# Tarseus/eam-rl4co

Measured on AMD Instinct MI355X. Metric: env-steps/sec (batch x num_loc / s), AttentionModel construction rollout, higher is better.
Workload: dtype f32; 1 GPU; TSP num_loc=100 batch=1024/GPU AM greedy rollout (encoder + cache + decode loop + reward); global_batch=1024, launch=hipGraph replay

## Files before the change

eam_rl4co_amd/csrc/encoder_fused.hip:

```cpp
#include "encoder_fused.hpp"

namespace eamrl {

constexpr int SA = 140;
constexpr int GA = 34;
constexpr int SQ = 66;

struct ALayout {
    float* HB;
    static constexpr int S = SA;
    __device__ float* col(int c) const { return HB + (c & 3) * GA + (c >> 2); }
    __device__ void store4(int row, int q4, float4 v) const
    {
        float* p = HB + row * SA + q4;
        p[0] = v.x; p[GA] = v.y; p[2 * GA] = v.z; p[3 * GA] = v.w;
    }
    __device__ float4 load4(int row, int q4) const
    {
        const float* p = HB + row * SA + q4;
        return make_float4(p[0], p[GA], p[2 * GA], p[3 * GA]);
    }
    __device__ void mirror(int, int, float) const {}
};

#ifdef EAMRL_STAMPS
__device__ unsigned long long g_enc_stamps[24];
#define ESTAMP(i) do { const unsigned long long now_ = __builtin_readcyclecounter(); st_acc[i] += now_ - st_t; st_t = now_; } while (0)
#else
#define ESTAMP(i) do { } while (0)
#endif

__device__ __forceinline__ f32x4 mfma4(float a, float b, f32x4 c) { return __builtin_amdgcn_mfma_f32_16x16x4f32(a, b, c, 0, 0, 0); }

typedef float f32x2v __attribute__((ext_vector_type(2)));
__device__ __forceinline__ float2 lds_read_b64(const float* p)
{
    typedef const volatile __attribute__((address_space(3))) f32x2v* lds_ptr;
    const f32x2v v = *(lds_ptr)(p);
    return make_float2(v.x, v.y);
}

template <int CT>
__device__ __forceinline__ void load_b0(float4 (&b0)[CT], const float* const (&wp)[CT])
{
#pragma unroll
    for (int ct = 0; ct < CT; ++ct) b0[ct] = *reinterpret_cast<const float4*>(wp[ct]);
}

template <int RTW, int CT, int S, bool SWAP, int NRT>
__device__ __forceinline__ void gemm_pass_n(f32x4 (&acc)[RTW][CT], const float* arow, const float* const (&wp)[CT],
                                            int NU, const float4 (&b0)[CT])
{
    constexpr int nrt = NRT;
    float4 bn[CT];
    float2 an0[RTW], an1[RTW];
#pragma unroll
    for (int ct = 0; ct < CT; ++ct) bn[ct] = b0[ct];
#pragma unroll
    for (int rt = 0; rt < RTW; ++rt)
        if (rt < nrt) {
            an0[rt] = lds_read_b64(arow + rt * 16 * S);
            an1[rt] = lds_read_b64(arow + rt * 16 * S + 2);
        }
    for (int u = 0; u < NU; ++u) {
        float4 b[CT];
        float2 a0[RTW], a1[RTW];
#pragma unroll
        for (int ct = 0; ct < CT; ++ct) b[ct] = bn[ct];
#pragma unroll
        for (int rt = 0; rt < RTW; ++rt) { a0[rt] = an0[rt]; a1[rt] = an1[rt]; }
        if (u + 1 < NU) {
#pragma unroll
            for (int ct = 0; ct < CT; ++ct) bn[ct] = *reinterpret_cast<const float4*>(wp[ct] + (u + 1) * 256);
#pragma unroll
            for (int rt = 0; rt < RTW; ++rt)
                if (rt < nrt) {
                    an0[rt] = lds_read_b64(arow + rt * 16 * S + 4 * (u + 1));
                    an1[rt] = lds_read_b64(arow + rt * 16 * S + 4 * (u + 1) + 2);
                }
        }
#pragma unroll
        for (int rt = 0; rt < RTW; ++rt)
            if (rt < nrt) {
#pragma unroll
                for (int ct = 0; ct < CT; ++ct)
                    acc[rt][ct] = SWAP ? mfma4(b[ct].x, a0[rt].x, acc[rt][ct]) : mfma4(a0[rt].x, b[ct].x, acc[rt][ct]);
#pragma unroll
                for (int ct = 0; ct < CT; ++ct)
                    acc[rt][ct] = SWAP ? mfma4(b[ct].y, a0[rt].y, acc[rt][ct]) : mfma4(a0[rt].y, b[ct].y, acc[rt][ct]);
#pragma unroll
                for (int ct = 0; ct < CT; ++ct)
                    acc[rt][ct] = SWAP ? mfma4(b[ct].z, a1[rt].x, acc[rt][ct]) : mfma4(a1[rt].x, b[ct].z, acc[rt][ct]);
#pragma unroll
                for (int ct = 0; ct < CT; ++ct)
                    acc[rt][ct] = SWAP ? mfma4(b[ct].w, a1[rt].y, acc[rt][ct]) : mfma4(a1[rt].y, b[ct].w, acc[rt][ct]);
            }
    }
}

template <int RTW, int CT, int S, bool SWAP = false, int NLOW = RTW>
__device__ __forceinline__ void gemm_pass(f32x4 (&acc)[RTW][CT], const float* arow, int nrt, const float* const (&wp)[CT],
                                          int NU, const float4 (&b0)[CT])
{
    if (NLOW == RTW || nrt == RTW) gemm_pass_n<RTW, CT, S, SWAP, RTW>(acc, arow, wp, NU, b0);
    else gemm_pass_n<RTW, CT, S, SWAP, NLOW>(acc, arow, wp, NU, b0);
}

template <int RTW>
__device__ __forceinline__ void residual_norm_store(const f32x4 (&acc)[RTW][2], float* HB, int row0, int nrt, int cw, int j, int G,
                                                    int norm, const float* cst )
{
#pragma unroll
    for (int ct = 0; ct < 2; ++ct) {
        const int c = 32 * cw + 16 * ct + j;
        const float sc = cst[c], sh = cst[FE + c];
        float* col = HB + (c & 3) * GA + (c >> 2);
#pragma unroll
        for (int rt = 0; rt < RTW; ++rt)
            if (rt < nrt) {
#pragma unroll
                for (int r = 0; r < 4; ++r) {
                    float* p = col + (row0 + 16 * rt + 4 * G + r) * SA;
                    float v = *p + acc[rt][ct][r];
                    if (norm == EAMRL_NORM_BATCH_EVAL) v = fma_(v, sc, sh);
                    *p = v;
                }
            }
    }
}

template <int RTT>
__global__ __launch_bounds__(512, 2) void k_encoder_fused(FusedArgs a)
{
    constexpr int RTA = (RTT + 1) / 2;
    constexpr int RTW = RTA;
    constexpr int ROWS = 16 * RTT;
    constexpr int SV = ROWS + 4;
    extern __shared__ __attribute__((aligned(16))) float lds[];
    float* HB = lds;
    float* QA = HB + ROWS * SA;
    float* KB = QA + ROWS * SQ;
    float* VT = KB + ROWS * SQ;
    float* HID = QA;
    float* CST = VT + 64 * SV;
    static_assert(ROWS * SA <= 2 * ROWS * SQ + 64 * SV, "HID must fit QA | KB | VT");
    const ALayout L{HB};

    const int tid = threadIdx.x, lane = tid & 63;
    const int wv = __builtin_amdgcn_readfirstlane(tid >> 6);
    const int cw = wv & 3, rw = wv >> 2;
    const int j = lane & 15, G = lane >> 4;
    const int M = a.M;
    const int row0 = rw ? 16 * RTA : 0;
    const int nrt = rw ? RTT - RTA : RTA;
    const int64_t inst = blockIdx.x;
#ifdef EAMRL_STAMPS
    unsigned long long st_acc[20] = {0, 0, 0, 0, 0, 0, 0, 0, 0, 0, 0, 0, 0, 0, 0, 0, 0, 0, 0, 0}, st_t = __builtin_readcyclecounter();
#endif

    if (a.h_in) load_h<ROWS>(a.h_in, M, L);
    else init_embedding<ROWS>(a.init, M, L);
    __syncthreads();
    ESTAMP(0);

    for (int layer = 0; layer < a.nlayers; ++layer) {
        const eamrl_encoder_layer& Ly = a.L[layer];
        for (int i = tid; i < NCST; i += blockDim.x) {
            float v;
            if (i < C_BO) v = Ly.bqkv[i];
            else if (i < C_B1) v = Ly.bo[i - C_BO];
            else if (i < C_B2) v = Ly.b1[i - C_B1];
            else if (i < C_N1) v = Ly.b2[i - C_B2];
            else {
                const bool second = i >= C_N2;
                const int k = (i - (second ? C_N2 : C_N1));
                const int c = k & (FE - 1);
                const float* gam = second ? Ly.n2_gamma : Ly.n1_gamma;
                const float* bet = second ? Ly.n2_beta : Ly.n1_beta;
                if (a.norm == EAMRL_NORM_BATCH_EVAL) {
                    const float* mean = second ? Ly.n2_mean : Ly.n1_mean;
                    const float* var = second ? Ly.n2_var : Ly.n1_var;
                    const float sc = gam[c] / __builtin_sqrtf(var[c] + a.eps);
                    const float ms = mean[c] * sc;
                    v = k < FE ? sc : bet[c] - ms;
                } else {
                    v = k < FE ? gam[c] : bet[c];
                }
            }
            CST[i] = v;
        }
        __syncthreads();
        f32x4 acc_o[RTW][2];
#pragma unroll
        for (int ct = 0; ct < 2; ++ct) {
            const float b = CST[C_BO + 32 * cw + 16 * ct + j];
#pragma unroll
            for (int rt = 0; rt < RTW; ++rt) acc_o[rt][ct] = splat4(b);
        }
        for (int hg = 0; hg < 2; ++hg) {
            const float* wp3[2];
            float4 b3[2];
#pragma unroll
            for (int ct = 0; ct < 2; ++ct)
                wp3[ct] = Ly.Wo + ((int64_t)(2 * cw + ct) * (FE / 16) + 4 * hg) * 256 + lane * 4;
            {
                f32x4 acc[RTW][3];
                const int ctq = 4 * hg + cw;
                const float* wp[3];
                float4 b0[3];
#pragma unroll
                for (int x = 0; x < 3; ++x) wp[x] = Ly.Wqkv + ((int64_t)(8 * x + ctq) * (FE / 16)) * 256 + lane * 4;
                load_b0<3>(b0, wp);
#pragma unroll
                for (int x = 0; x < 3; ++x) {
                    const float b = CST[C_BQKV + 16 * (8 * x + ctq) + j];
#pragma unroll
                    for (int rt = 0; rt < RTW; ++rt) acc[rt][x] = splat4(b);
                }
                ESTAMP(16);
                gemm_pass<RTW, 3, SA, false, RTT - RTA>(acc, HB + (row0 + j) * SA + G * GA, nrt, wp, FE / 16, b0);
                ESTAMP(17);
                load_b0<2>(b3, wp3);
                float* qcol = QA + (j & 3) * 16 + 4 * cw + (j >> 2);
                float* kcol = KB + (j & 3) * 16 + 4 * cw + (j >> 2);
                float* vrow = VT + (16 * cw + j) * SV;
#pragma unroll
                for (int rt = 0; rt < RTW; ++rt)
                    if (rt < nrt) {
                        const int rbase = row0 + 16 * rt + 4 * G;
#pragma unroll
                        for (int r = 0; r < 4; ++r) {
                            qcol[(rbase + r) * SQ] = acc[rt][0][r] * 0.25f;
                            kcol[(rbase + r) * SQ] = acc[rt][1][r];
                        }
                        *reinterpret_cast<float4*>(vrow + rbase) =
                            make_float4(acc[rt][2][0], acc[rt][2][1], acc[rt][2][2], acc[rt][2][3]);
                    }
            }
            ESTAMP(1);
            __syncthreads();
            ESTAMP(2);
            {
                const int pi = 4 * (j & 3) + (j >> 2);
                float kf[RTT][4];
#pragma unroll
                for (int kt = 0; kt < RTT; ++kt) {
                    const float* p = KB + (16 * kt + pi) * SQ + G * 16 + 4 * cw;
                    const float2 lo = *reinterpret_cast<const float2*>(p), hi = *reinterpret_cast<const float2*>(p + 2);
                    kf[kt][0] = lo.x; kf[kt][1] = lo.y; kf[kt][2] = hi.x; kf[kt][3] = hi.y;
                }
                float vf[4 * RTT];
                const int NT = (M + 3) >> 2;
                constexpr int FULLT = RTT == 7 ? 4 : RTT == 4 ? 2 : 0;
#pragma unroll
                for (int t = 0; t < 4 * RTT; ++t) vf[t] = (t < NT) ? VT[(16 * cw + j) * SV + 4 * t + G] : 0.0f;
                for (int q = 0; q < nrt; ++q) {
                    const int qrow = row0 + 16 * q + j;
                    const float* qp = QA + qrow * SQ + G * 16 + 4 * cw;
                    const float2 qlo = *reinterpret_cast<const float2*>(qp), qhi = *reinterpret_cast<const float2*>(qp + 2);
                    f32x4 s[RTT];
                    float m = -INFINITY;
#pragma unroll
                    for (int kt = 0; kt < RTT; ++kt) s[kt] = mfma4(kf[kt][0], qlo.x, splat4(0.0f));
#pragma unroll
                    for (int kt = 0; kt < RTT; ++kt) s[kt] = mfma4(kf[kt][1], qlo.y, s[kt]);
#pragma unroll
                    for (int kt = 0; kt < RTT; ++kt) s[kt] = mfma4(kf[kt][2], qhi.x, s[kt]);
#pragma unroll
                    for (int kt = 0; kt < RTT; ++kt) s[kt] = mfma4(kf[kt][3], qhi.y, s[kt]);
#pragma unroll
                    for (int kt = 0; kt < RTT; ++kt) {
                        if (kt >= FULLT && 16 * kt + 16 > M) {
#pragma unroll
                            for (int r = 0; r < 4; ++r)
                                if (16 * kt + 4 * r + G >= M) s[kt][r] = -INFINITY;
                        }
                        m = vmax5_raw(m, s[kt][0], s[kt][1], s[kt][2], s[kt][3]);
                    }
                    {
                        auto r16 = __builtin_amdgcn_permlane16_swap(__float_as_uint(m), __float_as_uint(m), false, false);
                        m = vmax_raw(__uint_as_float(r16[0]), __uint_as_float(r16[1]));
                        auto r32 = __builtin_amdgcn_permlane32_swap(__float_as_uint(m), __float_as_uint(m), false, false);
                        m = vmax_raw(__uint_as_float(r32[0]), __uint_as_float(r32[1]));
                    }
#pragma unroll
                    for (int kt = 0; kt < RTT; ++kt) {
                        f32x2 e01 = (f32x2){s[kt][0], s[kt][1]} - splat2(m), e23 = (f32x2){s[kt][2], s[kt][3]} - splat2(m);
                        d_expf2_nonpos_x2(e01, e23);
                        s[kt] = (f32x4){e01.x, e01.y, e23.x, e23.y};
                    }
                    float zp = s[0][0];
#pragma unroll
                    for (int t = 1; t < 4 * RTT; ++t) zp = zp + s[t >> 2][t & 3];
                    {
                        auto r16 = __builtin_amdgcn_permlane16_swap(__float_as_uint(zp), __float_as_uint(zp), false, false);
                        zp = __uint_as_float(r16[0]) + __uint_as_float(r16[1]);
                        auto r32 = __builtin_amdgcn_permlane32_swap(__float_as_uint(zp), __float_as_uint(zp), false, false);
                        zp = __uint_as_float(r32[0]) + __uint_as_float(r32[1]);
                    }
                    f32x4 o = splat4(0.0f);
#pragma unroll
                    for (int kt = 0; kt < RTT; ++kt)
                        if (kt < FULLT || 16 * kt < M) {
#pragma unroll
                            for (int r = 0; r < 4; ++r) o = mfma4(vf[4 * kt + r], s[kt][r], o);
                        }
                    float* op = QA + qrow * SQ + 4 * cw + G;
#pragma unroll
                    for (int r = 0; r < 4; ++r) op[r * 16] = o[r] / zp;
                }
            }
            ESTAMP(3);
            __syncthreads();
            ESTAMP(4);
            gemm_pass<RTW, 2, SQ, false, RTT - RTA>(acc_o, QA + (row0 + j) * SQ + G * 16, nrt, wp3, 4, b3);
            ESTAMP(5);
            __syncthreads();
            ESTAMP(6);
        }
        residual_norm_store<RTW>(acc_o, HB, row0, nrt, cw, j, G, a.norm, CST + C_N1);
        __syncthreads();
        if (a.norm == EAMRL_NORM_INSTANCE) {
            instance_norm(L, M, a.eps, CST + C_N1);
            __syncthreads();
        }
        ESTAMP(7);
        f32x4 acc_f[RTW][2];
#pragma unroll
        for (int ct = 0; ct < 2; ++ct) {
            const float b = CST[C_B2 + 32 * cw + 16 * ct + j];
#pragma unroll
            for (int rt = 0; rt < RTW; ++rt) acc_f[rt][ct] = splat4(b);
        }
        for (int ch = 0; ch < FF / 128; ++ch) {
            const float* wp5[2];
            float4 b5[2];
#pragma unroll
            for (int ct = 0; ct < 2; ++ct)
                wp5[ct] = Ly.W2 + ((int64_t)(2 * cw + ct) * (FF / 16) + 8 * ch) * 256 + lane * 4;
            {
                f32x4 acc[RTW][2];
                const float* wp[2];
                float4 b0[2];
#pragma unroll
                for (int ct = 0; ct < 2; ++ct) wp[ct] = Ly.W1 + ((int64_t)(8 * ch + 2 * cw + ct) * (FE / 16)) * 256 + lane * 4;
                load_b0<2>(b0, wp);
#pragma unroll
                for (int ct = 0; ct < 2; ++ct) {
                    const float b = CST[C_B1 + 16 * (8 * ch + 2 * cw + ct) + j];
#pragma unroll
                    for (int rt = 0; rt < RTW; ++rt) acc[rt][ct] = splat4(b);
                }
                ESTAMP(14);
                gemm_pass<RTW, 2, SA, false, RTT - RTA>(acc, HB + (row0 + j) * SA + G * GA, nrt, wp, FE / 16, b0);
                ESTAMP(15);
                load_b0<2>(b5, wp5);
#pragma unroll
                for (int ct = 0; ct < 2; ++ct) {
                    const int c = 32 * cw + 16 * ct + j;
                    float* col = HID + (c & 3) * GA + (c >> 2);
#pragma unroll
                    for (int rt = 0; rt < RTW; ++rt)
                        if (rt < nrt) {
#pragma unroll
                            for (int r = 0; r < 4; ++r) {
                                const float v = acc[rt][ct][r];
                                col[(row0 + 16 * rt + 4 * G + r) * SA] = !(v > 0.0f) ? 0.0f : v;
                            }
                        }
                }
            }
            ESTAMP(8);
            __syncthreads();
            ESTAMP(9);
            gemm_pass<RTW, 2, SA, false, RTT - RTA>(acc_f, HID + (row0 + j) * SA + G * GA, nrt, wp5, 8, b5);
            ESTAMP(10);
            __syncthreads();
            ESTAMP(11);
        }
        residual_norm_store<RTW>(acc_f, HB, row0, nrt, cw, j, G, a.norm, CST + C_N2);
        __syncthreads();
        if (a.norm == EAMRL_NORM_INSTANCE) {
            instance_norm(L, M, a.eps, CST + C_N2);
            __syncthreads();
        }
        ESTAMP(12);
    }
    if (a.h_out) store_h(a.h_out, M, L);
    ESTAMP(13);
    if (a.cache.gctx) graph_context(a.cache.Wg, a.cache.gctx, M, L, CST);
    if (a.cache.out) {
        float* STG = QA;
        float* crow = a.cache.out + (inst * (int64_t)M) * a.cache.ld;
        for (int sl = 0; sl <= a.cache.nproj; ++sl) {
            const bool lp = sl == a.cache.nproj;
            f32x4 acc[RTW][2];
            const float* wp[2];
            float4 b0[2];
#pragma unroll
            for (int ct = 0; ct < 2; ++ct)
                wp[ct] = (lp ? a.cache.WoutT : a.cache.Wc + (int64_t)sl * FE * FE) + ((int64_t)(2 * cw + ct) * (FE / 16)) * 256 + lane * 4;
            load_b0<2>(b0, wp);
#pragma unroll
            for (int ct = 0; ct < 2; ++ct)
#pragma unroll
                for (int rt = 0; rt < RTW; ++rt) acc[rt][ct] = splat4(0.0f);
            if (lp) __syncthreads();
            gemm_pass<RTW, 2, SA, true, RTT - RTA>(acc, (lp ? STG : HB) + (row0 + j) * SA + G * GA, nrt, wp, FE / 16, b0);
#pragma unroll
            for (int rt = 0; rt < RTW; ++rt)
                if (rt < nrt) {
                    const int node = row0 + 16 * rt + j;
#pragma unroll
                    for (int ct = 0; ct < 2; ++ct) {
                        const int c = 32 * cw + 16 * ct + 4 * G;
                        const f32x4 v = acc[rt][ct];
                        if (node < M)
                            *reinterpret_cast<float4*>(crow + (int64_t)node * a.cache.ld + sl * FE + c) = make_float4(v[0], v[1], v[2], v[3]);
                        if (sl == 2) {
                            float* p = STG + node * SA + (c >> 2);
                            p[0] = v[0]; p[GA] = v[1]; p[2 * GA] = v[2]; p[3 * GA] = v[3];
                        }
                    }
                }
        }
    }
#ifdef EAMRL_STAMPS
    if (lane == 0) {
        for (int i = 0; i < 20; ++i) atomicAdd(&g_enc_stamps[i], st_acc[i]);
        atomicAdd(&g_enc_stamps[20], 1ull);
    }
#endif
}

__global__ void k_pack_mfma_b(const float* __restrict__ W, float* __restrict__ Wp, int N, int K)
{
    const int64_t idx = (int64_t)blockIdx.x * blockDim.x + threadIdx.x;
    if (idx >= (int64_t)N * K) return;
    const int q = (int)(idx & 3), l = (int)((idx >> 2) & 63);
    const int64_t blk = idx >> 8;
    const int u = (int)(blk % (K / 16)), ct = (int)(blk / (K / 16));
    const int j = l & 15, g = l >> 4;
    Wp[idx] = W[(int64_t)(16 * ct + j) * K + 16 * u + 4 * q + g];
}

int launch_pack_mfma_b(const float* W, float* Wp, int N, int K, hipStream_t st)
{
    const int64_t n = (int64_t)N * K;
    hipLaunchKernelGGL(k_pack_mfma_b, dim3((unsigned)((n + 255) / 256)), dim3(256), 0, st, W, Wp, N, K);
    return hipGetLastError() == hipSuccess ? 0 : EAMRL_E_LAUNCH;
}

#ifdef EAMRL_STAMPS
extern "C" __attribute__((visibility("default"))) int eamrl_debug_read_enc_stamps(unsigned long long* out, int reset)
{
    if (hipMemcpyFromSymbol(out, HIP_SYMBOL(g_enc_stamps), sizeof(g_enc_stamps)) != hipSuccess) return -1;
    if (reset) {
        unsigned long long z[24] = {0};
        if (hipMemcpyToSymbol(HIP_SYMBOL(g_enc_stamps), z, sizeof(z)) != hipSuccess) return -1;
    }
    return 0;
}
#endif

bool encoder_fused_supports(int M, int E, int H, int FFdim, int nlayers)
{
    return M >= 1 && M <= 112 && E == FE && H == FH && FFdim == FF && nlayers >= 1 && nlayers <= MAX_FUSED_LAYERS;
}

int launch_encoder_fused(const float* h_in, float* h_out, int64_t B, int M, int nlayers, int norm, float eps,
                         const eamrl_encoder_layer* layers, const eamrl_encoder_cache* cache, const eamrl_encoder_init* init,
                         int dtype, hipStream_t st)
{
    if (B <= 0) return 0;
    FusedArgs a = {};
    a.h_in = init ? nullptr : h_in; a.h_out = h_out; a.M = M; a.nlayers = nlayers; a.norm = norm; a.eps = eps;
    if (cache) {
        a.cache = *cache;
        if (!cache->Wg || !cache->gctx) a.cache.Wg = a.cache.gctx = nullptr;
    }
    if (init) a.init = *init;
    for (int l = 0; l < nlayers; ++l) a.L[l] = layers[l];
    if (dtype != DTYPE_F32) return launch_encoder_fused16(a, B, dtype, st);
    return launch_fused(a, B, st, [](auto rtt) {
        constexpr int RTT = decltype(rtt)::value, ROWS = 16 * RTT;
        return FusedVariant{k_encoder_fused<RTT>, ((size_t)ROWS * SA + 2 * (size_t)ROWS * SQ + 64 * (size_t)(ROWS + 4) + NCST) * sizeof(float)};
    });
}

}
```

Before: 49.14 million env-steps/s.

## Software-pipeline encoder GEMM passes with prefetched operands and MFMA/load interleaving

The encoder GEMM inner loop becomes fully unrolled with a compile-time trip count and double-buffered A/B register fragments. sched_group_barrier hints interleave the global and LDS loads with the MFMAs. The first weight and activation fragments of the next GEMM (QKV for the next head group, W1 for the next FFN chunk) are now prefetched during the preceding pass or across barriers, hiding load latency at pass starts. Asm barriers on lane indices steer register allocation. The cost is higher register pressure and longer code, which may lower occupancy or cause spills.

```diff
diff --git a/eam_rl4co_amd/csrc/encoder_fused.hip b/eam_rl4co_amd/csrc/encoder_fused.hip
--- a/eam_rl4co_amd/csrc/encoder_fused.hip
+++ b/eam_rl4co_amd/csrc/encoder_fused.hip
@@ -40,76 +40,95 @@
     return make_float2(v.x, v.y);
 }
 
+__device__ __forceinline__ float4 global_load_b128(const float* p)
+{
+    typedef const __attribute__((address_space(1))) f32x4* global_ptr;
+    const f32x4 v = *(global_ptr)(p);
+    return make_float4(v[0], v[1], v[2], v[3]);
+}
+
 template <int CT>
 __device__ __forceinline__ void load_b0(float4 (&b0)[CT], const float* const (&wp)[CT])
 {
 #pragma unroll
-    for (int ct = 0; ct < CT; ++ct) b0[ct] = *reinterpret_cast<const float4*>(wp[ct]);
-}
-
-template <int RTW, int CT, int S, bool SWAP, int NRT>
-__device__ __forceinline__ void gemm_pass_n(f32x4 (&acc)[RTW][CT], const float* arow, const float* const (&wp)[CT],
-                                            int NU, const float4 (&b0)[CT])
-{
-    constexpr int nrt = NRT;
-    float4 bn[CT];
-    float2 an0[RTW], an1[RTW];
-#pragma unroll
-    for (int ct = 0; ct < CT; ++ct) bn[ct] = b0[ct];
+    for (int ct = 0; ct < CT; ++ct) b0[ct] = global_load_b128(wp[ct]);
+}
+
+template <int RTW, int S>
+__device__ __forceinline__ void load_a0(float2 (&a0)[RTW][2], const float* arow, int nrt)
+{
 #pragma unroll
     for (int rt = 0; rt < RTW; ++rt)
         if (rt < nrt) {
-            an0[rt] = lds_read_b64(arow + rt * 16 * S);
-            an1[rt] = lds_read_b64(arow + rt * 16 * S + 2);
-        }
+            a0[rt][0] = lds_read_b64(arow + rt * 16 * S);
+            a0[rt][1] = lds_read_b64(arow + rt * 16 * S + 2);
+        }
+}
+
+template <int RTW, int CT, int S, bool SWAP, int NRT, int NU>
+__device__ __forceinline__ void gemm_pass_n(f32x4 (&acc)[RTW][CT], const float* arow, const float* const (&wp)[CT],
+                                            const float4 (&b0)[CT], const float2 (&a0)[RTW][2])
+{
+    float4 b[2][CT];
+    float2 a[2][NRT][2];
+#pragma unroll
+    for (int ct = 0; ct < CT; ++ct) b[0][ct] = b0[ct];
+#pragma unroll
+    for (int rt = 0; rt < NRT; ++rt) { a[0][rt][0] = a0[rt][0]; a[0][rt][1] = a0[rt][1]; }
+#pragma unroll
     for (int u = 0; u < NU; ++u) {
-        float4 b[CT];
-        float2 a0[RTW], a1[RTW];
-#pragma unroll
-        for (int ct = 0; ct < CT; ++ct) b[ct] = bn[ct];
-#pragma unroll
-        for (int rt = 0; rt < RTW; ++rt) { a0[rt] = an0[rt]; a1[rt] = an1[rt]; }
+        const int c = u & 1, n = c ^ 1;
+        __builtin_amdgcn_sched_barrier(0);
         if (u + 1 < NU) {
 #pragma unroll
-            for (int ct = 0; ct < CT; ++ct) bn[ct] = *reinterpret_cast<const float4*>(wp[ct] + (u + 1) * 256);
-#pragma unroll
-            for (int rt = 0; rt < RTW; ++rt)
-                if (rt < nrt) {
-                    an0[rt] = lds_read_b64(arow + rt * 16 * S + 4 * (u + 1));
-                    an1[rt] = lds_read_b64(arow + rt * 16 * S + 4 * (u + 1) + 2);
-                }
-        }
-#pragma unroll
-        for (int rt = 0; rt < RTW; ++rt)
-            if (rt < nrt) {
-#pragma unroll
-                for (int ct = 0; ct < CT; ++ct)
-                    acc[rt][ct] = SWAP ? mfma4(b[ct].x, a0[rt].x, acc[rt][ct]) : mfma4(a0[rt].x, b[ct].x, acc[rt][ct]);
-#pragma unroll
-                for (int ct = 0; ct < CT; ++ct)
-                    acc[rt][ct] = SWAP ? mfma4(b[ct].y, a0[rt].y, acc[rt][ct]) : mfma4(a0[rt].y, b[ct].y, acc[rt][ct]);
-#pragma unroll
-                for (int ct = 0; ct < CT; ++ct)
-                    acc[rt][ct] = SWAP ? mfma4(b[ct].z, a1[rt].x, acc[rt][ct]) : mfma4(a1[rt].x, b[ct].z, acc[rt][ct]);
-#pragma unroll
-                for (int ct = 0; ct < CT; ++ct)
-                    acc[rt][ct] = SWAP ? mfma4(b[ct].w, a1[rt].y, acc[rt][ct]) : mfma4(a1[rt].y, b[ct].w, acc[rt][ct]);
-            }
-    }
-}
-
-template <int RTW, int CT, int S, bool SWAP = false, int NLOW = RTW>
+            for (int ct = 0; ct < CT; ++ct) b[n][ct] = global_load_b128(wp[ct] + (u + 1) * 256);
+#pragma unroll
+            for (int rt = 0; rt < NRT; ++rt) {
+                a[n][rt][0] = lds_read_b64(arow + rt * 16 * S + 4 * (u + 1));
+                a[n][rt][1] = lds_read_b64(arow + rt * 16 * S + 4 * (u + 1) + 2);
+            }
+        }
+#pragma unroll
+        for (int rt = 0; rt < NRT; ++rt) {
+#pragma unroll
+            for (int ct = 0; ct < CT; ++ct)
+                acc[rt][ct] = SWAP ? mfma4(b[c][ct].x, a[c][rt][0].x, acc[rt][ct]) : mfma4(a[c][rt][0].x, b[c][ct].x, acc[rt][ct]);
+#pragma unroll
+            for (int ct = 0; ct < CT; ++ct)
+                acc[rt][ct] = SWAP ? mfma4(b[c][ct].y, a[c][rt][0].y, acc[rt][ct]) : mfma4(a[c][rt][0].y, b[c][ct].y, acc[rt][ct]);
+#pragma unroll
+            for (int ct = 0; ct < CT; ++ct)
+                acc[rt][ct] = SWAP ? mfma4(b[c][ct].z, a[c][rt][1].x, acc[rt][ct]) : mfma4(a[c][rt][1].x, b[c][ct].z, acc[rt][ct]);
+#pragma unroll
+            for (int ct = 0; ct < CT; ++ct)
+                acc[rt][ct] = SWAP ? mfma4(b[c][ct].w, a[c][rt][1].y, acc[rt][ct]) : mfma4(a[c][rt][1].y, b[c][ct].w, acc[rt][ct]);
+        }
+        if (u + 1 < NU) {
+            __builtin_amdgcn_sched_group_barrier(0x20, CT, 0);
+#pragma unroll
+            for (int i = 0; i < 2 * NRT; ++i) {
+                __builtin_amdgcn_sched_group_barrier(0x8, 2, 0);
+                __builtin_amdgcn_sched_group_barrier(0x100, 1, 0);
+            }
+            __builtin_amdgcn_sched_group_barrier(0x8, 4 * NRT * (CT - 1), 0);
+        }
+    }
+    __builtin_amdgcn_sched_barrier(0);
+}
+
+template <int RTW, int CT, int S, int NU, bool SWAP = false, int NLOW = RTW>
 __device__ __forceinline__ void gemm_pass(f32x4 (&acc)[RTW][CT], const float* arow, int nrt, const float* const (&wp)[CT],
-                                          int NU, const float4 (&b0)[CT])
-{
-    if (NLOW == RTW || nrt == RTW) gemm_pass_n<RTW, CT, S, SWAP, RTW>(acc, arow, wp, NU, b0);
-    else gemm_pass_n<RTW, CT, S, SWAP, NLOW>(acc, arow, wp, NU, b0);
+                                          const float4 (&b0)[CT], const float2 (&a0)[RTW][2])
+{
+    if (NLOW == RTW || nrt == RTW) gemm_pass_n<RTW, CT, S, SWAP, RTW, NU>(acc, arow, wp, b0, a0);
+    else gemm_pass_n<RTW, CT, S, SWAP, NLOW, NU>(acc, arow, wp, b0, a0);
 }
 
 template <int RTW>
 __device__ __forceinline__ void residual_norm_store(const f32x4 (&acc)[RTW][2], float* HB, int row0, int nrt, int cw, int j, int G,
                                                     int norm, const float* cst )
 {
+    asm volatile("" : "+v"(j), "+v"(G));
 #pragma unroll
     for (int ct = 0; ct < 2; ++ct) {
         const int c = 32 * cw + 16 * ct + j;
@@ -154,6 +173,7 @@
     const int row0 = rw ? 16 * RTA : 0;
     const int nrt = rw ? RTT - RTA : RTA;
     const int64_t inst = blockIdx.x;
+    const float* hrow = HB + (row0 + j) * SA + G * GA;
 #ifdef EAMRL_STAMPS
     unsigned long long st_acc[20] = {0, 0, 0, 0, 0, 0, 0, 0, 0, 0, 0, 0, 0, 0, 0, 0, 0, 0, 0, 0}, st_t = __builtin_readcyclecounter();
 #endif
@@ -165,6 +185,13 @@
 
     for (int layer = 0; layer < a.nlayers; ++layer) {
         const eamrl_encoder_layer& Ly = a.L[layer];
+        const float* wp1[3];
+        float4 b1[3];
+        float2 a1[RTW][2];
+#pragma unroll
+        for (int x = 0; x < 3; ++x) wp1[x] = Ly.Wqkv + ((int64_t)(8 * x + cw) * (FE / 16)) * 256 + lane * 4;
+        load_b0<3>(b1, wp1);
+        load_a0<RTW, SA>(a1, hrow, nrt);
         for (int i = tid; i < NCST; i += blockDim.x) {
             float v;
             if (i < C_BO) v = Ly.bqkv[i];
@@ -206,11 +233,6 @@
             {
                 f32x4 acc[RTW][3];
                 const int ctq = 4 * hg + cw;
-                const float* wp[3];
-                float4 b0[3];
-#pragma unroll
-                for (int x = 0; x < 3; ++x) wp[x] = Ly.Wqkv + ((int64_t)(8 * x + ctq) * (FE / 16)) * 256 + lane * 4;
-                load_b0<3>(b0, wp);
 #pragma unroll
                 for (int x = 0; x < 3; ++x) {
                     const float b = CST[C_BQKV + 16 * (8 * x + ctq) + j];
@@ -218,16 +240,18 @@
                     for (int rt = 0; rt < RTW; ++rt) acc[rt][x] = splat4(b);
                 }
                 ESTAMP(16);
-                gemm_pass<RTW, 3, SA, false, RTT - RTA>(acc, HB + (row0 + j) * SA + G * GA, nrt, wp, FE / 16, b0);
+                gemm_pass<RTW, 3, SA, FE / 16, false, RTT - RTA>(acc, hrow, nrt, wp1, b1, a1);
                 ESTAMP(17);
                 load_b0<2>(b3, wp3);
-                float* qcol = QA + (j & 3) * 16 + 4 * cw + (j >> 2);
-                float* kcol = KB + (j & 3) * 16 + 4 * cw + (j >> 2);
-                float* vrow = VT + (16 * cw + j) * SV;
+                int je = j, Ge = G;
+                asm volatile("" : "+v"(je), "+v"(Ge));
+                float* qcol = QA + (je & 3) * 16 + 4 * cw + (je >> 2);
+                float* kcol = KB + (je & 3) * 16 + 4 * cw + (je >> 2);
+                float* vrow = VT + (16 * cw + je) * SV;
 #pragma unroll
                 for (int rt = 0; rt < RTW; ++rt)
                     if (rt < nrt) {
-                        const int rbase = row0 + 16 * rt + 4 * G;
+                        const int rbase = row0 + 16 * rt + 4 * Ge;
 #pragma unroll
                         for (int r = 0; r < 4; ++r) {
                             qcol[(rbase + r) * SQ] = acc[rt][0][r] * 0.25f;
@@ -241,11 +265,13 @@
             __syncthreads();
             ESTAMP(2);
             {
-                const int pi = 4 * (j & 3) + (j >> 2);
+                int jp = j, Gp = G;
+                asm volatile("" : "+v"(jp), "+v"(Gp));
+                const int pi = 4 * (jp & 3) + (jp >> 2);
                 float kf[RTT][4];
 #pragma unroll
                 for (int kt = 0; kt < RTT; ++kt) {
-                    const float* p = KB + (16 * kt + pi) * SQ + G * 16 + 4 * cw;
+                    const float* p = KB + (16 * kt + pi) * SQ + Gp * 16 + 4 * cw;
                     const float2 lo = *reinterpret_cast<const float2*>(p), hi = *reinterpret_cast<const float2*>(p + 2);
                     kf[kt][0] = lo.x; kf[kt][1] = lo.y; kf[kt][2] = hi.x; kf[kt][3] = hi.y;
                 }
@@ -253,10 +279,10 @@
                 const int NT = (M + 3) >> 2;
                 constexpr int FULLT = RTT == 7 ? 4 : RTT == 4 ? 2 : 0;
 #pragma unroll
-                for (int t = 0; t < 4 * RTT; ++t) vf[t] = (t < NT) ? VT[(16 * cw + j) * SV + 4 * t + G] : 0.0f;
+                for (int t = 0; t < 4 * RTT; ++t) vf[t] = (t < NT) ? VT[(16 * cw + jp) * SV + 4 * t + Gp] : 0.0f;
                 for (int q = 0; q < nrt; ++q) {
-                    const int qrow = row0 + 16 * q + j;
-                    const float* qp = QA + qrow * SQ + G * 16 + 4 * cw;
+                    const int qrow = row0 + 16 * q + jp;
+                    const float* qp = QA + qrow * SQ + Gp * 16 + 4 * cw;
                     const float2 qlo = *reinterpret_cast<const float2*>(qp), qhi = *reinterpret_cast<const float2*>(qp + 2);
                     f32x4 s[RTT];
                     float m = -INFINITY;
@@ -273,7 +299,7 @@
                         if (kt >= FULLT && 16 * kt + 16 > M) {
 #pragma unroll
                             for (int r = 0; r < 4; ++r)
-                                if (16 * kt + 4 * r + G >= M) s[kt][r] = -INFINITY;
+                                if (16 * kt + 4 * r + Gp >= M) s[kt][r] = -INFINITY;
                         }
                         m = vmax5_raw(m, s[kt][0], s[kt][1], s[kt][2], s[kt][3]);
                     }
@@ -305,7 +331,7 @@
 #pragma unroll
                             for (int r = 0; r < 4; ++r) o = mfma4(vf[4 * kt + r], s[kt][r], o);
                         }
-                    float* op = QA + qrow * SQ + 4 * cw + G;
+                    float* op = QA + qrow * SQ + 4 * cw + Gp;
 #pragma unroll
                     for (int r = 0; r < 4; ++r) op[r * 16] = o[r] / zp;
                 }
@@ -313,17 +339,32 @@
             ESTAMP(3);
             __syncthreads();
             ESTAMP(4);
-            gemm_pass<RTW, 2, SQ, false, RTT - RTA>(acc_o, QA + (row0 + j) * SQ + G * 16, nrt, wp3, 4, b3);
+            float2 a3[RTW][2];
+            load_a0<RTW, SQ>(a3, QA + (row0 + j) * SQ + G * 16, nrt);
+            if (hg == 0) {
+#pragma unroll
+                for (int x = 0; x < 3; ++x) wp1[x] += 4 * (FE / 16) * 256;
+                load_b0<3>(b1, wp1);
+                load_a0<RTW, SA>(a1, hrow, nrt);
+            }
+            gemm_pass<RTW, 2, SQ, 4, false, RTT - RTA>(acc_o, QA + (row0 + j) * SQ + G * 16, nrt, wp3, b3, a3);
             ESTAMP(5);
             __syncthreads();
             ESTAMP(6);
         }
+        const float* wp4[2];
+        float4 b4[2];
+        float2 a4[RTW][2];
+#pragma unroll
+        for (int ct = 0; ct < 2; ++ct) wp4[ct] = Ly.W1 + ((int64_t)(2 * cw + ct) * (FE / 16)) * 256 + lane * 4;
+        load_b0<2>(b4, wp4);
         residual_norm_store<RTW>(acc_o, HB, row0, nrt, cw, j, G, a.norm, CST + C_N1);
         __syncthreads();
         if (a.norm == EAMRL_NORM_INSTANCE) {
             instance_norm(L, M, a.eps, CST + C_N1);
             __syncthreads();
         }
+        load_a0<RTW, SA>(a4, hrow, nrt);
         ESTAMP(7);
         f32x4 acc_f[RTW][2];
 #pragma unroll
@@ -340,11 +381,6 @@
                 wp5[ct] = Ly.W2 + ((int64_t)(2 * cw + ct) * (FF / 16) + 8 * ch) * 256 + lane * 4;
             {
                 f32x4 acc[RTW][2];
-                const float* wp[2];
-                float4 b0[2];
-#pragma unroll
-                for (int ct = 0; ct < 2; ++ct) wp[ct] = Ly.W1 + ((int64_t)(8 * ch + 2 * cw + ct) * (FE / 16)) * 256 + lane * 4;
-                load_b0<2>(b0, wp);
 #pragma unroll
                 for (int ct = 0; ct < 2; ++ct) {
                     const float b = CST[C_B1 + 16 * (8 * ch + 2 * cw + ct) + j];
@@ -352,7 +388,7 @@
                     for (int rt = 0; rt < RTW; ++rt) acc[rt][ct] = splat4(b);
                 }
                 ESTAMP(14);
-                gemm_pass<RTW, 2, SA, false, RTT - RTA>(acc, HB + (row0 + j) * SA + G * GA, nrt, wp, FE / 16, b0);
+                gemm_pass<RTW, 2, SA, FE / 16, false, RTT - RTA>(acc, hrow, nrt, wp4, b4, a4);
                 ESTAMP(15);
                 load_b0<2>(b5, wp5);
 #pragma unroll
@@ -373,7 +409,15 @@
             ESTAMP(8);
             __syncthreads();
             ESTAMP(9);
-            gemm_pass<RTW, 2, SA, false, RTT - RTA>(acc_f, HID + (row0 + j) * SA + G * GA, nrt, wp5, 8, b5);
+            float2 a5[RTW][2];
+            load_a0<RTW, SA>(a5, HID + (row0 + j) * SA + G * GA, nrt);
+            if (ch + 1 < FF / 128) {
+#pragma unroll
+                for (int ct = 0; ct < 2; ++ct) wp4[ct] += 8 * (FE / 16) * 256;
+                load_b0<2>(b4, wp4);
+                load_a0<RTW, SA>(a4, hrow, nrt);
+            }
+            gemm_pass<RTW, 2, SA, 8, false, RTT - RTA>(acc_f, HID + (row0 + j) * SA + G * GA, nrt, wp5, b5, a5);
             ESTAMP(10);
             __syncthreads();
             ESTAMP(11);
@@ -406,7 +450,10 @@
 #pragma unroll
                 for (int rt = 0; rt < RTW; ++rt) acc[rt][ct] = splat4(0.0f);
             if (lp) __syncthreads();
-            gemm_pass<RTW, 2, SA, true, RTT - RTA>(acc, (lp ? STG : HB) + (row0 + j) * SA + G * GA, nrt, wp, FE / 16, b0);
+            const float* arow = (lp ? STG : HB) + (row0 + j) * SA + G * GA;
+            float2 a0[RTW][2];
+            load_a0<RTW, SA>(a0, arow, nrt);
+            gemm_pass<RTW, 2, SA, FE / 16, true, RTT - RTA>(acc, arow, nrt, wp, b0, a0);
 #pragma unroll
             for (int rt = 0; rt < RTW; ++rt)
                 if (rt < nrt) {
```

Result: faster. 50.27 million env-steps/s (median of 6 runs) (+2.3%).
